# VanshJP/ShippingEnv

Measured on AMD Instinct MI355X. Metric: env-steps/sec at N=2^20 parallel envs per GPU (config 3: full step, 5 default ports; K steps in the steady state after a 1000-step pre-roll; config3_literal: the survey's 1000 steps from reset), higher is better.
Workload: dtype f64+int (fuel f64; reward computed in f64, stored f32 after one rounding; positions/cargo int)

## Files before the change

### shippingenv_amd/csrc/shipenv.hip

```cpp
#include <hip/hip_runtime.h>

#include <math.h>
#include <stdint.h>
#include <stdio.h>
#include <stdlib.h>
#include <string.h>

#include <algorithm>
#include <atomic>
#include <initializer_list>
#include <string>
#include <vector>

#include "../../include/shipenv.h"
#include "navfield.h"
#include "philox.h"
#include "step_lean.h"

#ifndef SHIPENV_TRACE
#define SHIPENV_TRACE 0
#endif

using namespace shipenv;

// ... 157 lines not shown
        double r = 0.0;
        if (k & 4) r += -10.0;
        if (k & 2) {
            r += -5.0;
        } else {
            r += -0.0001;
            r += -1.0;
        }
        r += (k & 1) ? 2.0 : -2.0;
        rtab[k] = r;
    }
    rtab[8] = 0.05;
    rtab[9] = 0.0;
    memcpy(&img[d.rtab()], rtab, sizeof rtab);
    dims = d;
    if (distinct) *distinct = ports_on_distinct_cells(P, px, py);
    return SE_OK;
}

int upload_world(se_env* env, int32_t P, const int32_t* px, const int32_t* py, const int32_t* pf,
                 const int32_t* pc) {
    WorldDims d{};
    std::vector<uint32_t> img;
    bool distinct = false;
    int rc = build_world_image(env->dims.H, env->dims.W, env->water, P, px, py, pf, pc, d, img, &distinct);
    if (rc) return rc;
    std::vector<uint8_t> ring(ring_table_bytes(d.H, d.W));
    ring_table_build(d.H, d.W, reinterpret_cast<const uint8_t*>(img.data()), ring.data());
    rc = device_reserve(env->d_world, env->world_cap, (size_t)d.padded() * 4 + ring.size());
    if (rc) return rc;
    HIP_TRY(hipMemcpy(env->d_world, img.data(), (size_t)d.padded() * 4, hipMemcpyHostToDevice));
    HIP_TRY(hipMemcpy(env->d_world + d.padded(), ring.data(), ring.size(), hipMemcpyHostToDevice));
    env->dims = d;
    env->ports_distinct = distinct;
    env->port_x.assign(px, px + P);
    env->port_y.assign(py, py + P);
    env->cmax = env->fmax = env->stock_cargo_max = 0;
    for (int i = 0; i < P; ++i) {
        env->cmax = std::max(env->cmax, std::min(pc[i], 49));
        env->fmax = std::max(env->fmax, std::min(pf[i], 199));
        env->stock_cargo_max = std::max(env->stock_cargo_max, pc[i]);
    }
    env->world_version += 1;
    env->mask_ntmpl = 1 + P;
    for (int p = 0; p < P; ++p)
        for (int q = 0; q < P; ++q) env->mask_ntmpl += (px[p] == px[q] && py[p] == py[q]) ? 1 : 0;
    return SE_OK;
}

typedef void (*StepFn)(StepArgs);
struct StepRow {
    uint32_t key;
    StepFn fn;
};
constexpr uint32_t step_key(bool typed, bool replay, bool autoreset, bool nt = false, bool rec = false, bool seq = false) {
    return typed | replay << 1 | autoreset << 2 | nt << 3 | rec << 4 | seq << 5;
}
template <bool... kFlags>
constexpr StepRow step_row() {
    return {step_key(kFlags...), step_kernel<kFlags...>};
}
template <bool... kFlags>
constexpr StepRow tail_row() {
    return {step_key(kFlags...), step_tail_kernel<kFlags...>};
}
constexpr StepRow kStepKernels[] = {
    step_row<false, false, false>(), step_row<false, false, false, true>(),
    step_row<false, false, true>(), step_row<false, false, true, true>(),
    step_row<false, false, false, false, false, true>(),
    step_row<false, false, false, true, false, true>(),
    step_row<false, false, true, false, true>(), step_row<false, false, true, true, true>(),
    step_row<false, true, false>(), step_row<true, true, false>(),
    step_row<true, false, false>(), step_row<true, false, true>(),
};
constexpr StepRow kStepTailKernels[] = {
    tail_row<false, false, false>(), tail_row<false, false, true>(), tail_row<false, true, false>(),
    tail_row<true, true, false>(),   tail_row<true, false, false>(), tail_row<true, false, true>(),
};

template <size_t kRows>
StepFn find_kernel(const StepRow (&rows)[kRows], uint32_t key) {
    for (const StepRow& r : rows)
        if (r.key == key) return r.fn;
    return nullptr;
}

StepArgs step_args(const se_env* env, const int32_t* act) {
    StepArgs A{};
    A.world = env->d_world;
    A.dims = env->dims;
    A.n = env->n;
    A.env_base = env->env_base;
    A.seed = env->seed;
    A.t = (uint32_t)env->step_t;
    A.st = env->st;
    A.act = act;
    A.iters = env->iters;
    return A;
}

int launch_step(se_env* env, bool typed, bool replay, const int32_t* act, const int32_t* a,
                const int32_t* b, se_tape* tape, void* stream, const StepRecord* rec = nullptr,
                bool seq = false) {
    int rc = check_ready(env);
    if (rc) return rc;
    if (env->n > 0 && (!act || (typed && (!a || !b)) || (replay && !tape)))
        return fail(SE_EINVAL, "null action/tape pointer");
    if (!aligned16(act) || (typed && (!aligned16(a) || !aligned16(b))))
        return fail(SE_EINVAL, "action buffers must be 16-byte aligned");
    const bool autoreset = (env->flags & SE_FLAG_AUTO_RESET) && !replay;
    if (autoreset && env->dims.P < 2) return fail(SE_EINVAL, "auto-reset needs at least two ports");
    DeviceGuard g(env->device);
    StepArgs A = step_args(env, act);
    A.act_a = a;
    A.act_b = b;
    A.tape = tape;
    if (autoreset) {
        const size_t par = (size_t)(env->step_t & 1u);
        A.done_recs = env->st.done_recs + par * (size_t)env->nseg * (size_t)env->seg;
        A.done_count = env->st.done_count + par * (size_t)env->nseg;
    }
    A.seg = env->seg;
    A.done_pad = env->done_pad;
    A.slab = env->d_slab;
    if (rec) A.rec = *rec;
    const bool agent = !typed && !replay;
    const StepFn full = find_kernel(kStepKernels, step_key(typed, replay, autoreset, agent && env->nt_loads,
                                                           rec != nullptr, agent && !autoreset && seq));
    const StepFn tail = find_kernel(kStepTailKernels, step_key(typed, replay, autoreset));
    if (!full || !tail) return fail(SE_EINVAL, "no step kernel for this kind of step");
    const hipStream_t s = (hipStream_t)stream;
    if (env->n >= kEnvsPerThread) {
        full<<<env->grid, kStepBlock, lds_bytes(env), s>>>(A);
        HIP_TRY(hipGetLastError());
    }
    if (env->n & 3) {
        tail<<<1, 64, 0, s>>>(A);
        HIP_TRY(hipGetLastError());
    }
    if (!replay) env->step_t += 1;
    return SE_OK;
}

int launch_step_seq(se_env* env, const int32_t* act, int64_t ld, int32_t steps, void* stream) {
    if (!act) return fail(SE_EINVAL, "null action/tape pointer");
    if (!aligned16(act)) return fail(SE_EINVAL, "action buffers must be 16-byte aligned");
    DeviceGuard g(env->device);
    const StepArgs A = step_args(env, act);
    const hipStream_t s = (hipStream_t)stream;
    if (env->n >= kEnvsPerThread) {
        const size_t base = lds_bytes(env) + kStockByCodeBytes;
        const bool pool = env->seq_gate_pool && base + kGatePoolBytes <= kLdsDefault;
        const size_t without = base + (pool ? kGatePoolBytes : 0);
        const uint32_t ring = env->seq_ring && ring_table_fits(env->dims.H, env->dims.W, env->dims.P, without)
                                  ? ring_table_bytes(env->dims.H, env->dims.W) : 0u;
        const size_t lds = without + ring;
        const auto kernel = pool ? (env->nt_loads ? step_seq_kernel<true, true> : step_seq_kernel<false, true>)
                                 : (env->nt_loads ? step_seq_kernel<true, false> : step_seq_kernel<false, false>);
        kernel<<<env->grid, kStepBlock, lds, s>>>(A, steps, ld, ring | (arrive_by_code_allowed(env->dims.P, env->ports_distinct) ? kSeqDistinctPorts : 0u), env->seq_screen ? 0u : ~0u);
        HIP_TRY(hipGetLastError());
    }
    if (env->n & 3) {
        step_tail_seq_kernel<<<1, 64, 0, s>>>(A, steps, ld);
        HIP_TRY(hipGetLastError());
    }
    env->step_t += (uint64_t)steps;
    return SE_OK;
}

int launch_reset(se_env* env, const uint8_t* mask, const int32_t* origin, const int32_t* dest, void* stream) {
    if (env->n == 0) return SE_OK;
    DeviceGuard g(env->device);
    const ResetArgs A{env->d_world, env->dims, env->n, env->env_base, env->seed,
                      (uint32_t)env->epoch, (uint32_t)env->step_t, env->st, mask, origin, dest};
    reset_kernel<<<grid_for(env->n), kBlock, 0, (hipStream_t)stream>>>(A);
    HIP_TRY(hipGetLastError());
    return SE_OK;
}

}

void shipenv_set_error(const std::string& msg) { g_err = msg; }

extern "C" {

#if SHIPENV_TRACE
extern "C" int se_trace_read(void* host, size_t bytes) {
    return hipMemcpyFromSymbol(host, HIP_SYMBOL(g_trace), bytes) == hipSuccess ? 0 : -1;
}
#endif

int se_abi_version(void) { return SHIPENV_ABI_VERSION; }

const char* se_last_error(void) { return g_err.c_str(); }

int se_create(se_env** out, int device, int64_t n, int64_t env_id_base, int32_t H, int32_t W,
              const uint8_t* water, int32_t P, const int32_t* port_x, const int32_t* port_y,
              const int32_t* port_fuel, const int32_t* port_cargo, uint64_t seed, uint32_t flags) {
    if (!out) return fail(SE_EINVAL, "null out");
    *out = nullptr;
    if (n < 0) return fail(SE_EINVAL, "n must be >= 0");
    if (env_id_base < 0 || (env_id_base & 3))
        return fail(SE_EINVAL, "env_id_base must be a multiple of 4 (envs 4k..4k+3 share draw blocks)");
    if (H < 1 || W < 1 || H > SE_MAX_SIDE || W > SE_MAX_SIDE)
        return fail(SE_EINVAL, "map sides must be in [1, 256]");
    if (!water) return fail(SE_EINVAL, "null water map");
    if (P > 0 && (!port_x || !port_y || !port_fuel || !port_cargo))
        return fail(SE_EINVAL, "null port arrays");
    int ndev = 0;
    HIP_TRY(hipGetDeviceCount(&ndev));
    if (device < 0 || device >= ndev) return fail(SE_EINVAL, "bad device ordinal");
    DeviceGuard g(device);
    se_env* env = new se_env();
    env->device = device;
    env->n = n;
    env->env_base = env_id_base;
    env->seed = seed;
    env->flags = flags;
    env->dims.H = H;
    env->dims.W = W;
    env->water.assign(water, water + (size_t)H * W);
    for (auto& v : env->water) v = v ? 1 : 0;
    int rc = upload_world(env, P, port_x, port_y, port_fuel, port_cargo);
    if (rc) {
        se_destroy(env);
        return rc;
    }
    {
        const int64_t groups = (n + kEnvsPerThread - 1) / kEnvsPerThread;
        const int64_t cap = step_block_cap();
        env->iters = groups > 0 ? (groups + cap * kStepBlock - 1) / (cap * kStepBlock) : 1;
        env->grid = (int)(groups > 0 ? (groups + env->iters * kStepBlock - 1) / (env->iters * kStepBlock) : 1);
        env->seg = 64 * kEnvsPerThread;
        env->nseg = (int64_t)env->grid * env->iters * (kStepBlock / 64);
        env->nslab = (int64_t)env->grid * (kStepBlock / 64);
        env->done_pad = done_pad_records(env);
        env->nt_loads = step_nt_loads(env);
        env->seq_fuse = seq_fuse();
        env->seq_max_steps = seq_max_steps();
        env->seq_gate_pool = seq_gate_pool();
        env->seq_ring = seq_ring();
        env->seq_screen = seq_screen();
        env->mask_tiled = mask_tiled();
    }
    hipError_t e = hipMalloc(&env->d_slab, (size_t)env->nslab * 4 * sizeof(double));
    if (e == hipSuccess) e = hipMemset(env->d_slab, 0, (size_t)env->nslab * 4 * sizeof(double));
    if (e != hipSuccess) {
        se_destroy(env);
        return fail(SE_EHIP, std::string("se_create allocation: ") + hipGetErrorString(e));
    }
    *out = env;
    return SE_OK;
}

int se_set_ports(se_env* env, int32_t P, const int32_t* port_x, const int32_t* port_y,
                 const int32_t* port_fuel, const int32_t* port_cargo) {
    if (!env) return fail(SE_EINVAL, "null env");
    if (P > 0 && (!port_x || !port_y || !port_fuel || !port_cargo))
        return fail(SE_EINVAL, "null port arrays");
    DeviceGuard g(env->device);
    HIP_TRY(hipDeviceSynchronize());
    return upload_world(env, P, port_x, port_y, port_fuel, port_cargo);
}

int se_bind(se_env* env, const se_state* st) {
    if (!env || !st) return fail(SE_EINVAL, "null argument");
    const void* req[] = {st->x, st->y, st->fuel, st->cargo, st->origin, st->dest,
                         st->reward, st->done, st->err};
    for (const void* p : req) {
        if (!p && env->n > 0) return fail(SE_EINVAL, "null state buffer");
        if (!aligned16(p)) return fail(SE_EINVAL, "state buffers must be 16-byte aligned");
    }
    if (env->flags & SE_FLAG_AUTO_RESET) {
        if ((env->n > 0 && (!st->ep_return || !st->ep_start)) || !st->done_recs || !st->done_count)
            return fail(SE_EINVAL, "auto-reset needs ep_return, ep_start, done_recs and done_count");
        if (!aligned16(st->ep_return) || !aligned16(st->ep_start) || !aligned16(st->done_recs))
            return fail(SE_EINVAL, "state buffers must be 16-byte aligned");
        DeviceGuard g(env->device);
        HIP_TRY(hipMemset(st->done_count, 0, 2 * (size_t)env->nseg * sizeof(int32_t)));
    }
    env->st = *st;
    env->bound = true;
    return SE_OK;
}

int se_reset(se_env* env, const uint8_t* mask, void* stream) {
    int rc = check_ready(env);
    if (rc) return rc;
    if (env->dims.P < 2) return fail(SE_EINVAL, "reset needs at least two ports");
    rc = launch_reset(env, mask, nullptr, nullptr, stream);
    if (rc) return rc;
    env->epoch += 1;
    return SE_OK;
}

int se_reset_to(se_env* env, const uint8_t* mask, const int32_t* origin, const int32_t* dest,
                void* stream) {
    int rc = check_ready(env);
    if (rc) return rc;
    if (env->n > 0 && (!origin || !dest)) return fail(SE_EINVAL, "null origin/dest");
    return launch_reset(env, mask, origin, dest, stream);
}

int se_step(se_env* env, const int32_t* actions, void* stream) {
    return launch_step(env, false, false, actions, nullptr, nullptr, nullptr, stream);
}

int se_step_seq_mark(se_env* env, const int32_t* actions, int64_t ld, int32_t steps, void* stream,
                     void* event, int32_t mark_after) {
    int rc = check_ready(env);
    if (rc) return rc;
    if (steps < 0) return fail(SE_EINVAL, "negative step count");
// ... 341 lines not shown
```

### shippingenv_amd/csrc/step_lean.h

```cpp
#pragma once
#include <hip/hip_runtime.h>
#include <math.h>
#include <stdint.h>

namespace shipenv {

__host__ __device__ __forceinline__ bool lean_do_move(int act, int P, bool nodest, bool inb) {
    const bool is_mv = (uint32_t)act + 4u < (P != 0 ? 8u : 0u);
    return is_mv & !nodest & inb;
}
__host__ __device__ __forceinline__ uint32_t lean_move_bound(int P) {
    return P != 0 ? 0xFFFFFFF7u : 0xFFFFFFFFu;
}
__host__ __device__ __forceinline__ bool lean_do_move_val(int val, uint32_t bound, bool nodest, bool inb) {
    const bool is_mv = (uint32_t)val > bound;
    return is_mv & !nodest & inb;
}
__host__ __device__ __forceinline__ bool lean_sel_ok(int act, int P, bool same) {
    const bool is_sel = (uint32_t)act - 4u < (uint32_t)P;
    return is_sel & !same;
}

constexpr uint32_t kRingBorder = 254;
constexpr uint32_t kRingGround = 255;
constexpr int kRingMaxPorts = 253;
constexpr size_t kRingLdsPerBlock = 160 * 1024 / 4;
constexpr uint32_t kRingBias = 0x00010001u;

__host__ __device__ __forceinline__ uint32_t ring_table_bytes(int H, int W) {
    return ((uint32_t)(H + 2) * (uint32_t)(W + 2) + 15u) & ~15u;
}
__host__ __device__ __forceinline__ bool ring_table_fits(int H, int W, int P, size_t lds_without) {
    return P <= kRingMaxPorts && lds_without + ring_table_bytes(H, W) <= kRingLdsPerBlock;
}
__host__ __forceinline__ void ring_table_build(int H, int W, const uint8_t* cell, uint8_t* out) {
    const uint32_t n = ring_table_bytes(H, W);
    for (uint32_t i = 0; i < n; ++i) out[i] = i < (uint32_t)(H + 2) * (uint32_t)(W + 2) ? (uint8_t)kRingBorder : 0;
    for (int x = 0; x < H; ++x)
        for (int y = 0; y < W; ++y) out[(size_t)(x + 1) * (size_t)(W + 2) + (size_t)(y + 1)] = cell[(size_t)x * W + y];
}
__host__ __device__ __forceinline__ uint32_t ring_bias(uint32_t p) { return p + kRingBias; }
__host__ __device__ __forceinline__ uint32_t ring_unbias(uint32_t bp) { return bp - kRingBias; }
__host__ __device__ __forceinline__ uint32_t ring_index(uint32_t bp, int W) {
    return (bp & 0xffffu) * (uint32_t)(W + 2) + (bp >> 16);
}
__host__ __device__ __forceinline__ bool ring_do_move(int val, uint32_t bound, uint32_t code) {
    return ((uint32_t)val > bound) & (code != kRingBorder);
}
__host__ __device__ __forceinline__ bool ring_moved(int val, uint32_t bound, uint32_t code) {
    return ((uint32_t)val > bound) & (code < kRingBorder);
}

__host__ __device__ __forceinline__ double lean_fuel(double fuel, double scale, bool moved) {
    return __builtin_fma(-scale, moved ? 1.0 : 0.0, fuel);
}

__host__ __device__ __forceinline__ double lean_fuel_scale(uint32_t w, double fifth) {
    return 1.0 + __builtin_fma((double)w, fifth, -0.1);
}

__host__ __device__ __forceinline__ uint32_t gate_window_log2(uint32_t m) {
    return m <= 8 ? 3u : m <= 16 ? 2u : 1u;
}

constexpr uint32_t kGatePoolLimit = 16;
constexpr uint32_t kGatePoolSeeds = 32;
constexpr uint32_t kGatePoolRow = 64 + kGatePoolSeeds;
constexpr uint32_t kGateWindowMax = 16;
constexpr uint32_t gate_window_entry_of(uint32_t m) {
    return m == 0 ? kGateWindowMax : (64u / m < kGateWindowMax ? 64u / m : kGateWindowMax) | ((65535u / m + 1u) << 8);
}
__host__ __device__ __forceinline__ uint32_t gate_window_entry(uint32_t m) {
    constexpr auto e = gate_window_entry_of;
    static constexpr uint32_t tab[17] = {e(0), e(1), e(2), e(3), e(4), e(5), e(6), e(7), e(8), e(9), e(10), e(11), e(12), e(13), e(14), e(15), e(16)};
    return tab[m];
}
__host__ __device__ __forceinline__ uint32_t gate_window_len(uint32_t entry) { return entry & 0xffu; }
__host__ __device__ __forceinline__ uint32_t gate_lane_offset(uint32_t L, uint32_t entry) { return (L * (entry >> 8)) >> 16; }
__host__ __device__ __forceinline__ uint32_t gate_lane_carrier(uint32_t L, uint32_t offset, uint32_t m) { return L - offset * m; }
__host__ __device__ __forceinline__ uint32_t gate_pool_index(uint32_t s, uint32_t m, uint32_t slot) { return s * m + slot; }
constexpr bool gate_pool_reads_in_rows() {
    for (uint32_t m = 1; m <= kGatePoolLimit; ++m) {
        const uint32_t W = gate_window_entry_of(m) & 0xffu;
        if (W < 4 || W > kGateWindowMax || m * W > 64 || (W - 1u) * m + m >= kGatePoolRow) return false;
    }
    return true;
}
__host__ __device__ __forceinline__ uint64_t gate_screen_mask(uint32_t m) { return m != 0 ? (1ull << m) - 1ull : ~0ull; }
__host__ __device__ __forceinline__ bool gate_screen_step(uint64_t shifted, uint64_t mask) { return (shifted & mask) != 0; }

__host__ __forceinline__ bool ports_on_distinct_cells(int P, const int32_t* px, const int32_t* py) {
    for (int i = 0; i < P; ++i)
        for (int k = 0; k < i; ++k)
            if (px[i] == px[k] && py[i] == py[k]) return false;
    return true;
}
__host__ __forceinline__ bool arrive_by_code_allowed(int P, bool distinct) { return distinct && P >= 2; }
__host__ __device__ __forceinline__ bool arrive_by_code(bool do_move, uint32_t code, int dst) {
    return do_move & (code == (uint32_t)dst + 1u);
}

__host__ __forceinline__ uint32_t gate_thr_entry(int c, double max_cargo) {
    return c < (int)max_cargo ? (uint32_t)floor(ldexp((double)c / max_cargo, 32)) : 0xffffffffu;
}

__host__ __device__ __forceinline__ bool screen_hot(const uint32_t word[4], const uint32_t thr[4]) {
    return (word[0] <= thr[0]) | (word[1] <= thr[1]) | (word[2] <= thr[2]) | (word[3] <= thr[3]);
}
__host__ __device__ __forceinline__ uint32_t screen_fold(uint64_t ballot, uint32_t logw) {
    uint32_t b = (uint32_t)ballot | (uint32_t)(ballot >> 32);
    b |= b >> 16;
    b |= b >> 8;
    b |= logw < 3u ? b >> 4 : 0u;
    b |= logw < 2u ? b >> 2 : 0u;
    return b;
}

}
```

### shippingenv_amd/csrc/step_seq.h

```cpp
#pragma once

#ifndef SHIPENV_SEQ_WINDOW_DIV
#define SHIPENV_SEQ_WINDOW_DIV 1
#endif
#ifndef SHIPENV_SEQ_CARGO_CUT
#define SHIPENV_SEQ_CARGO_CUT 1
#endif
#ifndef SHIPENV_SEQ_ARRIVE_CODE
#define SHIPENV_SEQ_ARRIVE_CODE 1
#endif

struct Carried {
    uint32_t pos[4];
    int org[4], dst[4];
    uint32_t code[4];
    bool near;
    bool bycode;
    uint32_t thr[4];
    const int2* take;
};
__device__ __forceinline__ uint32_t gate_thr_of(const LdsWorld& w, int cargo) {
    return w.gate_thr[min(max(cargo, 0), 50)];
}
template <bool kSched>
struct SeqInv {
    KeySched ks;
    uint32_t move_bound;
    uint32_t ring0;
    __device__ __forceinline__ U4 block(const Key& qk, uint32_t t, uint32_t slot) const {
        if constexpr (kSched) return draw_sched(ks, qk, t, slot);
        else return draw(qk, t, slot);
    }
};
struct NoLateDraw {
    __device__ __forceinline__ void operator()(U4&) const {}
};
template <bool kNt, bool kSched, typename Late = NoLateDraw>
__device__ __forceinline__ bool step_group_state(const LdsWorld& w, const SeqInv<kSched>& I, const Key& qk, uint32_t t, U4 fb,
                                                 const U4& gb, Group<false, false, kNt>& G, Carried& U, Late late = Late{}) {
    const int P = w.P;
    const uint32_t lim = (uint32_t)(w.H - 1) | ((uint32_t)(w.W - 1) << 16);
    const uint32_t wh = (uint32_t)w.W | (1u << 16);
    const uint32_t pm1 = P > 0 ? (uint32_t)(P - 1) : 0u;
    bool take_any = false;
#pragma unroll
    for (int j = 0; j < 4; ++j) take_any |= (G.a[j] >= 4 + P) & (U.code[j] != 0);
    const bool take_ran = __builtin_amdgcn_ballot_w64(take_any) != 0;
    if (take_ran) {
#pragma unroll
        for (int j = 0; j < 4; ++j) {
            const int act = G.a[j];
            const bool lt_tc = act < 54 + P;
            const int amount = act - (lt_tc ? 4 + P : 54 + P);
            const int2 st2 = U.take[U.code[j]];
            const int stock = lt_tc ? st2.y : st2.x;
            const bool ok_take = (act >= 4 + P) & (amount > 0) & (amount <= stock);
            G.c[j] = (ok_take & lt_tc) ? G.c[j] + amount : G.c[j];
            G.f[j] = (ok_take & !lt_tc) ? G.f[j] + (double)amount : G.f[j];
            U.thr[j] = gate_thr_of(w, G.c[j]);
        }
    }
    late(fb);
    uint32_t pos[4], cp[4], code_cp[4];
    int dst[4], cg[4];
    bool do_move[4], moved[4], inb[4], nodest[4];
#pragma unroll
    for (int j = 0; j < 4; ++j) {
        const uint32_t dxy = w.moves[G.a[j] & 3];
        const uint32_t p = U.pos[j];
        dst[j] = U.dst[j];
        const uint32_t np = pk_add_u16(p, dxy);
        inb[j] = pk_min_u16(np, lim) == np;
        nodest[j] = dst[j] == SE_NONE;
        cp[j] = (!nodest[j] & inb[j]) ? np : p;
        code_cp[j] = lds_cell(lds_address(w.cell), cp[j], wh);
    }
    asm("" : "+v"(code_cp[0]), "+v"(code_cp[1]), "+v"(code_cp[2]), "+v"(code_cp[3]));
#pragma unroll
    for (int j = 0; j < 4; ++j) {
        const int act = G.a[j];
        const int val = (int)((uint32_t)act - 4u);
        const uint32_t p = U.pos[j];
        cg[j] = G.c[j];
        const bool ground = code_cp[j] == kCellGround;
        const bool same = U.org[j] == val;
        do_move[j] = lean_do_move_val(val, I.move_bound, nodest[j], inb[j]);
        moved[j] = do_move[j] & !ground;
        const bool sel_ok = lean_sel_ok(act, P, same);
        pos[j] = moved[j] ? cp[j] : p;
        U.code[j] = moved[j] ? code_cp[j] : U.code[j];
        dst[j] = sel_ok ? val : dst[j];
    }
    uint32_t fire = 0, arrive = 0;
    bool arrive_any = false;
#pragma unroll
    for (int j = 0; j < 4; ++j) arrive_any |= do_move[j] & (U.code[j] != 0);
    if (__builtin_amdgcn_ballot_w64(arrive_any) != 0) {
#pragma unroll
        for (int j = 0; j < 4; ++j)
            arrive |= (uint32_t)(do_move[j] & (pos[j] == w.pos[min((uint32_t)dst[j], pm1)])) << j;
    }
    double f[4];
#pragma unroll
    for (int j = 0; j < 4; ++j) {
        f[j] = lean_fuel(G.f[j], lean_fuel_scale(fb.v[j], kFifthPerWord), moved[j]);
        const bool fires = do_move[j] & (cg[j] > 0) & (gb.v[j] <= U.thr[j]);
        fire |= (uint32_t)fires << j;
    }
    asm volatile("" : "+v"(fire), "+v"(arrive));
    int org[4];
#pragma unroll
    for (int j = 0; j < 4; ++j) {
        org[j] = U.org[j];
        U.pos[j] = pos[j];
        G.f[j] = f[j];
    }
    if (fire) {
        uint32_t lt[4], v1[4], v2[4], v3[4];
        const uint32_t rk[4] = {0u, fire & 1u, (uint32_t)__popc(fire & 3u), (uint32_t)__popc(fire & 7u)};
        U4 rr = I.block(qk, t, loss_slot(0));
#pragma unroll
        for (int j = 0; j < 4; ++j) {
            lt[j] = rr.v[0];
            v1[j] = rr.v[1];
            v2[j] = rr.v[2];
            v3[j] = rr.v[3];
        }
#pragma unroll
        for (uint32_t q = 1; q < 4; ++q) {
            if (__popc(fire) > q) {
                rr = I.block(qk, t, loss_slot(q));
#pragma unroll
                for (int j = (int)q; j < 4; ++j) {
                    const bool take = rk[j] >= q;
                    lt[j] = take ? rr.v[0] : lt[j];
                    v1[j] = take ? rr.v[1] : v1[j];
                    v2[j] = take ? rr.v[2] : v2[j];
                    v3[j] = take ? rr.v[3] : v3[j];
                }
            }
        }
#pragma unroll
        for (int j = 0; j < 4; ++j) {
            if (__builtin_amdgcn_ballot_w64((fire >> j) & 1u) == 0) continue;
            const uint32_t lo = min(v1[j], v2[j]), hi = max(v1[j], v2[j]);
            const uint32_t med = max(lo, min(hi, v3[j]));
            const int part = beta_part(med, cg[j]);
            const int some = lt[j] > kTypeHi ? cg[j] : part;
            const int loss = lt[j] < kTypeLo ? 0 : some;
            const bool fj = (fire >> j) & 1u;
            cg[j] = fj ? cg[j] - loss : cg[j];
            U.thr[j] = gate_thr_of(w, cg[j]);
        }
    }
    if (arrive) {
        const U4 ab = I.block(qk, t, kSlotArrive);
#pragma unroll
        for (int j = 0; j < 4; ++j) {
            const bool aj = (arrive >> j) & 1u;
            const int nd = pick_other(ab.v[j], P, dst[j]);
            cg[j] = aj ? 0 : cg[j];
            U.thr[j] = gate_thr_of(w, cg[j]);
            org[j] = aj ? dst[j] : org[j];
            dst[j] = aj ? nd : dst[j];
        }
    }
#pragma unroll
    for (int j = 0; j < 4; ++j) {
        U.org[j] = org[j];
        U.dst[j] = dst[j];
        G.c[j] = cg[j];
    }
    return take_ran;
}

struct GateDrawn {
    static constexpr bool kScreened = false;
    const U4& gb;
    __device__ __forceinline__ bool hot() const { return true; }
    __device__ __forceinline__ U4 words() const { return gb; }
};
__device__ __forceinline__ uint32_t here(uint32_t v) {
    asm volatile("" : "+v"(v));
    return v;
}
template <typename Read>
struct GateScreened {
    static constexpr bool kScreened = true;
    bool is_hot;
    Read read;
    __device__ __forceinline__ bool hot() const { return is_hot; }
    __device__ __forceinline__ U4 words() const { return read(); }
};
template <bool kNt, bool kSched, typename Gate, typename Late = NoLateDraw>
__device__ __forceinline__ bool step_group_ring(const LdsWorld& w, const SeqInv<kSched>& I, const Key& qk, uint32_t t, U4 fb,
                                                const Gate& gate, Group<false, false, kNt>& G, Carried& U, Late late = Late{}) {
    const int P = w.P;
    const uint32_t wh = (uint32_t)(w.W + 2) | (1u << 16);
    const uint32_t pm1 = P > 0 ? (uint32_t)(P - 1) : 0u;
    bool take_ran = false;
    if (U.near) {
        bool take_any = false;
#pragma unroll
        for (int j = 0; j < 4; ++j) take_any |= (G.a[j] >= 4 + P) & (U.code[j] != 0);
        take_ran = __builtin_amdgcn_ballot_w64(take_any) != 0;
        if (take_ran) {
            bool rose = false;
#pragma unroll
            for (int j = 0; j < 4; ++j) {
                const int act = G.a[j];
                const bool lt_tc = act < 54 + P;
                const int amount = act - (lt_tc ? 4 + P : 54 + P);
                const int2 st2 = U.take[U.code[j]];
                const int stock = lt_tc ? st2.y : st2.x;
                const bool ok_take = (act >= 4 + P) & (amount > 0) & (amount <= stock);
                rose |= ok_take & lt_tc;
                G.c[j] = (ok_take & lt_tc) ? G.c[j] + amount : G.c[j];
                G.f[j] = (ok_take & !lt_tc) ? G.f[j] + (double)amount : G.f[j];
                U.thr[j] = gate_thr_of(w, G.c[j]);
            }
#if SHIPENV_SEQ_CARGO_CUT
            take_ran = __builtin_amdgcn_ballot_w64(rose) != 0;
#else
            (void)rose;
#endif
        }
    }
    late(fb);
    uint32_t np[4], code_t[4];
#pragma unroll
    for (int j = 0; j < 4; ++j) {
        np[j] = pk_add_u16(U.pos[j], w.moves[G.a[j] & 3]);
        code_t[j] = lds_cell(I.ring0, np[j], wh);
    }
    asm("" : "+v"(code_t[0]), "+v"(code_t[1]), "+v"(code_t[2]), "+v"(code_t[3]));
    int dst[4], cg[4];
    bool do_move[4], moved[4], fires[4];
    double f[4];
#pragma unroll
    for (int j = 0; j < 4; ++j) {
        const int act = G.a[j];
        const int val = (int)((uint32_t)act - 4u);
        cg[j] = G.c[j];
        const bool same = U.org[j] == val;
        if constexpr (!Gate::kScreened) do_move[j] = ring_do_move(val, I.move_bound, code_t[j]);
        moved[j] = ring_moved(val, I.move_bound, code_t[j]);
        const bool sel_ok = lean_sel_ok(act, P, same);
        U.pos[j] = moved[j] ? np[j] : U.pos[j];
        U.code[j] = moved[j] ? code_t[j] : U.code[j];
        dst[j] = sel_ok ? val : U.dst[j];
        f[j] = lean_fuel(G.f[j], lean_fuel_scale(fb.v[j], kFifthPerWord), moved[j]);
        if constexpr (!Gate::kScreened) fires[j] = do_move[j] & (cg[j] > 0) & (gate.words().v[j] <= U.thr[j]);
    }
    const bool near = __builtin_amdgcn_ballot_w64((U.code[0] | U.code[1] | U.code[2] | U.code[3]) != 0) != 0;
    U.near = near;
    uint32_t arrive = 0;
    if (near) {
#pragma unroll
        for (int j = 0; j < 4; ++j)
            if constexpr (Gate::kScreened) do_move[j] = ring_do_move((int)((uint32_t)G.a[j] - 4u), I.move_bound, here(code_t[j]));
#if SHIPENV_SEQ_ARRIVE_CODE
        if (U.bycode) {
#pragma unroll
            for (int j = 0; j < 4; ++j) arrive |= (uint32_t)arrive_by_code(do_move[j], U.code[j], dst[j]) << j;
        } else
#endif
        {
#pragma unroll
            for (int j = 0; j < 4; ++j) arrive |= (uint32_t)(do_move[j] & (U.pos[j] == ring_bias(w.pos[min((uint32_t)dst[j], pm1)]))) << j;
        }
    }
    int org[4];
#pragma unroll
    for (int j = 0; j < 4; ++j) {
        org[j] = U.org[j];
        G.f[j] = f[j];
    }
    bool any_fire = false;
    if constexpr (Gate::kScreened) {
        if (gate.hot()) {
            const U4 gb = gate.words();
#pragma unroll
            for (int j = 0; j < 4; ++j)
                fires[j] = ring_do_move((int)((uint32_t)G.a[j] - 4u), I.move_bound, here(code_t[j])) & (cg[j] > 0) & (gb.v[j] <= U.thr[j]);
            any_fire = __builtin_amdgcn_ballot_w64(fires[0] | fires[1] | fires[2] | fires[3]) != 0;
        }
    } else {
        any_fire = __builtin_amdgcn_ballot_w64(fires[0] | fires[1] | fires[2] | fires[3]) != 0;
    }
    if (any_fire) {
        uint32_t fire = 0;
#pragma unroll
        for (int j = 0; j < 4; ++j) fire |= (uint32_t)fires[j] << j;
        asm volatile("" : "+v"(fire));
        uint32_t lt[4], v1[4], v2[4], v3[4];
        const uint32_t rk[4] = {0u, fire & 1u, (uint32_t)__popc(fire & 3u), (uint32_t)__popc(fire & 7u)};
        U4 rr = I.block(qk, t, loss_slot(0));
#pragma unroll
        for (int j = 0; j < 4; ++j) {
            lt[j] = rr.v[0];
            v1[j] = rr.v[1];
            v2[j] = rr.v[2];
            v3[j] = rr.v[3];
        }
#pragma unroll
        for (uint32_t q = 1; q < 4; ++q) {
            if (__popc(fire) > q) {
                rr = I.block(qk, t, loss_slot(q));
#pragma unroll
                for (int j = (int)q; j < 4; ++j) {
                    const bool take = rk[j] >= q;
                    lt[j] = take ? rr.v[0] : lt[j];
                    v1[j] = take ? rr.v[1] : v1[j];
                    v2[j] = take ? rr.v[2] : v2[j];
                    v3[j] = take ? rr.v[3] : v3[j];
                }
            }
        }
#pragma unroll
        for (int j = 0; j < 4; ++j) {
            if (__builtin_amdgcn_ballot_w64((fire >> j) & 1u) == 0) continue;
            const uint32_t lo = min(v1[j], v2[j]), hi = max(v1[j], v2[j]);
            const uint32_t med = max(lo, min(hi, v3[j]));
            const int part = beta_part(med, cg[j]);
            const int some = lt[j] > kTypeHi ? cg[j] : part;
            const int loss = lt[j] < kTypeLo ? 0 : some;
            const bool fj = (fire >> j) & 1u;
            cg[j] = fj ? cg[j] - loss : cg[j];
            U.thr[j] = gate_thr_of(w, cg[j]);
        }
    }
    if (arrive) {
        const U4 ab = I.block(qk, t, kSlotArrive);
#pragma unroll
        for (int j = 0; j < 4; ++j) {
            const bool aj = (arrive >> j) & 1u;
            const int nd = pick_other(ab.v[j], P, dst[j]);
            cg[j] = aj ? 0 : cg[j];
            U.thr[j] = gate_thr_of(w, cg[j]);
            org[j] = aj ? dst[j] : org[j];
            dst[j] = aj ? nd : dst[j];
        }
    }
#pragma unroll
    for (int j = 0; j < 4; ++j) {
        U.org[j] = org[j];
        U.dst[j] = dst[j];
        G.c[j] = cg[j];
    }
    return take_ran;
}

constexpr size_t kStockByCodeBytes = 256 * sizeof(int2);
static_assert(kStepBlock == 256, "stock_by_code: one cell code per thread");
__device__ __forceinline__ void stock_by_code(const LdsWorld& w, int2* take) {
    const uint32_t k = threadIdx.x - 1u, P = (uint32_t)w.P;
    const int2 s = w.stock[min(k, P > 0 ? P - 1 : 0u)];
    take[threadIdx.x] = k < P ? s : make_int2(0, 0);
}

constexpr uint32_t kGateDirectRun = 16;
constexpr uint32_t kGateEarlyCut = 2;
constexpr uint32_t kSeqDistinctPorts = 1;
static_assert(gate_pool_reads_in_rows(), "GATE pool: a window's reads lie in the wave's rows");
constexpr size_t kGatePoolBytes = (kStepBlock / 64) * kGatePoolRow * sizeof(uint4);
constexpr int kRingRows = 3;
static_assert(kGatePoolLimit <= kGatePoolSeeds && kGatePoolLimit <= 32, "GATE pool: a window of at least 2 steps");
static_assert(2 * kGatePoolLimit <= kGatePoolSeeds, "GATE pool: the carriers' threshold rows follow their seed rows");

template <bool kOpaque>
__device__ __forceinline__ uint32_t seq_lane() {
    uint32_t lane = threadIdx.x;
    if constexpr (kOpaque) asm volatile("" : "+v"(lane));
    return lane;
}

template <bool kNt, bool kPool>
__global__ __launch_bounds__(kStepBlock) __attribute__((amdgpu_waves_per_eu(4))) void step_seq_kernel(
    StepArgs A, int32_t steps, int64_t ld, uint32_t ring_bytes, uint32_t screen_all) {
    extern __shared__ uint32_t lds[];
    if (steps <= 0) return;
    const uint32_t ring16 = steps > 1 ? ring_bytes >> 4 : 0u;
    const bool has_ring = ring16 != 0;
    [[maybe_unused]] const bool distinct = (ring_bytes & kSeqDistinctPorts) != 0;
    const int64_t full = A.n >> 2;
    const int64_t first = (int64_t)blockIdx.x * A.iters * kStepBlock;

    const Staged st = stage_issue(A.world);
    __builtin_amdgcn_sched_barrier(0);
    Group<false, false, kNt> G;
    {
        const int64_t last = full - 1 - first;
        const uint32_t lane = last < (int64_t)threadIdx.x ? (uint32_t)(last < 0 ? 0 : last) : threadIdx.x;
        G.template load<true>(A, At<true>{last < 0 ? full - 1 : first, 0, A.n}, lane);
    }
    const uint4* const ring_g = reinterpret_cast<const uint4*>(A.world + A.dims.padded());
    const uint32_t ring_last = max(ring16, 1u) - 1u;
    const uint4 ring_r0 = ring_g[min(threadIdx.x, ring_last)];
    const uint4 ring_r1 = ring_g[min(threadIdx.x + kStepBlock, ring_last)];
    const uint4 ring_r2 = ring_g[min(threadIdx.x + 2 * kStepBlock, ring_last)];
    __builtin_amdgcn_sched_barrier(0);
    const LdsWorld w = stage_finish(A.world, A.dims, lds, st);
    int2* const take = reinterpret_cast<int2*>(lds + A.dims.padded());
    uint4* const gate_pool = reinterpret_cast<uint4*>(take + 256);
    uint4* const ring_l = reinterpret_cast<uint4*>(reinterpret_cast<uint8_t*>(take + 256) + (kPool ? kGatePoolBytes : 0));
    if (steps > 1) {
        stock_by_code(w, take);
        if (has_ring) {
            if (threadIdx.x < ring16) ring_l[threadIdx.x] = ring_r0;
            if (threadIdx.x + kStepBlock < ring16) ring_l[threadIdx.x + kStepBlock] = ring_r1;
            if (threadIdx.x + 2 * kStepBlock < ring16) ring_l[threadIdx.x + 2 * kStepBlock] = ring_r2;
            for (uint32_t i = threadIdx.x + kStepBlock * kRingRows; i < ring16; i += kStepBlock) ring_l[i] = ring_g[i];
        }
        __syncthreads();
    }

    SeqInv<kPool> I;
    if (steps > 1) {
        I.move_bound = lean_move_bound(w.P);
        asm volatile("" : "+s"(I.move_bound));
        I.ring0 = lds_address(reinterpret_cast<const uint8_t*>(ring_l));
    }

    BlockStats bs;
    Finished F;
    for (int64_t i = 0; i < A.iters; ++i) {
        const int64_t g0 = first + i * kStepBlock, g = g0 + threadIdx.x;
        if (g >= full) break;
        if (i > 0) {
            uint32_t lane = threadIdx.x;
            asm volatile("" : "+v"(lane));
            G.template load<true>(A, At<true>{g0, 0, A.n}, lane);
        }
        const uint32_t tl = A.t + (uint32_t)(steps - 1);
        if (steps > 1) {
            Carried U;
#pragma unroll
            for (int j = 0; j < 4; ++j) {
                U.pos[j] = unpack_pos(G.x, G.y, j);
                U.org[j] = byte_of(G.org, j);
                U.dst[j] = byte_of(G.dst, j);
                U.code[j] = w.cell[cell_of(U.pos[j], (uint32_t)w.W | (1u << 16))];
                U.thr[j] = gate_thr_of(w, G.c[j]);
            }
            U.take = take;
            bool irregular = false;
            {
                const uint32_t lim = (uint32_t)(w.H - 1) | ((uint32_t)(w.W - 1) << 16);
#pragma unroll
                for (int j = 0; j < 4; ++j) irregular |= (U.dst[j] == SE_NONE) | (pk_min_u16(U.pos[j], lim) != U.pos[j]);
            }
            const bool ring = has_ring && __builtin_amdgcn_ballot_w64(irregular) == 0;
            U.near = __builtin_amdgcn_ballot_w64((U.code[0] | U.code[1] | U.code[2] | U.code[3]) != 0) != 0;
            U.bycode = false;
#if SHIPENV_SEQ_ARRIVE_CODE
            if (distinct) {
                bool past = false;
#pragma unroll
                for (int j = 0; j < 4; ++j) past |= (uint32_t)U.dst[j] >= (uint32_t)w.P;
                U.bycode = __builtin_amdgcn_ballot_w64(past) == 0;
            }
#endif
            if (ring) {
#pragma unroll
                for (int j = 0; j < 4; ++j) U.pos[j] = ring_bias(U.pos[j]);
            }
            const Key qk = env_key(A.seed, (A.env_base + g * 4) >> 2);
            PairInv inv = pair_invariants(qk);
            asm volatile("" : "+v"(inv.hi[0]), "+v"(inv.lo[0]), "+v"(inv.hi[1]), "+v"(inv.lo[1]));
            const int32_t* row = A.act;
            if (!ring) {
                SeqInv<false> Ig;
                Ig.move_bound = I.move_bound;
                const uint32_t lane = seq_lane<kPool>();
                for (uint32_t t = A.t; t != tl; ++t) {
                    row += ld;
                    int32_t nxt[4];
                    ld4_full<kNt>(row, g0, nxt, lane);
                    const U4x2 fg = draw2(qk, inv, t);
                    step_group_state(w, Ig, qk, t, fg.fuel, fg.gate, G, U);
#pragma unroll
                    for (int j = 0; j < 4; ++j) G.a[j] = nxt[j];
                }
            } else if constexpr (!kPool) {
                for (uint32_t t = A.t; t != tl; ++t) {
                    row += ld;
                    int32_t nxt[4];
                    ld4_full<kNt>(row, g0, nxt);
                    const U4x2 fg = draw2(qk, inv, t);
                    step_group_ring(w, I, qk, t, fg.fuel, GateDrawn{fg.gate}, G, U);
#pragma unroll
                    for (int j = 0; j < 4; ++j) G.a[j] = nxt[j];
                }
            } else {
                {
                    const Key sk = env_key(A.seed, 0);
                    I.ks = key_schedule(sk.k0, sk.k1);
                    pin_schedule(I.ks);
                }
                const uint32_t lane = seq_lane<true>(), L = lane & 63u;
                uint4* const pool = gate_pool + (lane >> 6) * kGatePoolRow;
                uint4* const seeds = pool + 64;
                const bool whole = __builtin_amdgcn_ballot_w64(true) == ~0ull;
                uint32_t cuts = 0;
                for (uint32_t t = A.t; t != tl;) {
                    bool pooled = true;
                    do {
                        const bool carry = (G.c[0] > 0) | (G.c[1] > 0) | (G.c[2] > 0) | (G.c[3] > 0);
                        const uint64_t M = __builtin_amdgcn_ballot_w64(carry);
                        const uint32_t m = (uint32_t)__popcll(M);
                        if (!whole || m > kGatePoolLimit || (cuts >= 2 && m != 0)) {
                            pooled = false;
                            break;
                        }
                        const uint32_t slot = __builtin_amdgcn_mbcnt_hi((uint32_t)(M >> 32), __builtin_amdgcn_mbcnt_lo((uint32_t)M, 0u));
#if SHIPENV_SEQ_WINDOW_DIV
                        const uint32_t went = gate_window_entry(m);
                        uint64_t screen = (uint64_t)(int64_t)(int32_t)screen_all;
                        const uint64_t smask = gate_screen_mask(m);
                        if (m != 0) {
                            if (carry) {
                                seeds[slot] = make_uint4(inv.c3, inv.hi[1], inv.lo[1], qk.e1);
                                seeds[kGatePoolLimit + slot] = make_uint4(U.thr[0], U.thr[1], U.thr[2], U.thr[3]);
                            }
                            __builtin_amdgcn_fence(__ATOMIC_RELEASE, "wavefront");
                            __builtin_amdgcn_wave_barrier();
                            __builtin_amdgcn_fence(__ATOMIC_ACQUIRE, "wavefront");
                            const uint32_t so = gate_lane_offset(L, went), of = gate_lane_carrier(L, so, m);
                            const uint4 sd = seeds[of];
                            const uint4 th = seeds[kGatePoolLimit + of];
                            const U4 gw = draw_gate_pooled_sched(I.ks, GateSeed{sd.x, sd.y, sd.z, sd.w}, t + so);
                            pool[L] = make_uint4(gw.v[0], gw.v[1], gw.v[2], gw.v[3]);
                            screen |= __builtin_amdgcn_ballot_w64(gw.v[0] <= th.x) | __builtin_amdgcn_ballot_w64(gw.v[1] <= th.y) |
                                      __builtin_amdgcn_ballot_w64(gw.v[2] <= th.z) | __builtin_amdgcn_ballot_w64(gw.v[3] <= th.w);
                            __builtin_amdgcn_fence(__ATOMIC_RELEASE, "wavefront");
                            __builtin_amdgcn_wave_barrier();
                            __builtin_amdgcn_fence(__ATOMIC_ACQUIRE, "wavefront");
                        }
                        const uint32_t win = m != 0 ? min(tl - t, gate_window_len(went)) : tl - t;
                        uint32_t s = 0;
                        bool took;
                        do {
                            row += ld;
                            int32_t nxt[4];
                            ld4_full<kNt>(row, g0, nxt, lane);
                            const auto words = [&]() {
                                uint32_t so = s;
                                asm volatile("" : "+s"(so));
                                const uint4 g4 = pool[gate_pool_index(so, m, slot)];
                                return U4{{g4.x, g4.y, g4.z, g4.w}};
                            };
                            const auto fuel = [&](U4& fb) {
                                fb = draw_fuel_sched(I.ks, qk, inv, t);
                                asm volatile("" : "+v"(fb.v[0]), "+v"(fb.v[1]), "+v"(fb.v[2]), "+v"(fb.v[3]));
                            };
                            took = step_group_ring(w, I, qk, t, U4{}, GateScreened<decltype(words)>{gate_screen_step(screen, smask), words}, G, U, fuel);
#pragma unroll
                            for (int j = 0; j < 4; ++j) G.a[j] = nxt[j];
                            screen >>= m;
                            ++s;
                            ++t;
                        } while (!took && s != win);
#else
                        const uint32_t logw = gate_window_log2(m);
                        const uint32_t wmask = (1u << logw) - 1u;
                        uint32_t screen = screen_all;
                        if (m != 0) {
                            if (carry) {
                                seeds[slot] = make_uint4(inv.c3, inv.hi[1], inv.lo[1], qk.e1);
                                seeds[kGatePoolLimit + slot] = make_uint4(U.thr[0], U.thr[1], U.thr[2], U.thr[3]);
                            }
                            __builtin_amdgcn_fence(__ATOMIC_RELEASE, "wavefront");
                            __builtin_amdgcn_wave_barrier();
                            __builtin_amdgcn_fence(__ATOMIC_ACQUIRE, "wavefront");
                            const uint32_t of = min(L >> logw, m - 1u);
                            const uint4 sd = seeds[of];
                            const uint4 th = seeds[kGatePoolLimit + of];
                            const U4 gw = draw_gate_pooled_sched(I.ks, GateSeed{sd.x, sd.y, sd.z, sd.w}, t + (L & wmask));
                            pool[L] = make_uint4(gw.v[0], gw.v[1], gw.v[2], gw.v[3]);
                            const uint64_t hot = __builtin_amdgcn_ballot_w64(gw.v[0] <= th.x) | __builtin_amdgcn_ballot_w64(gw.v[1] <= th.y) |
                                                 __builtin_amdgcn_ballot_w64(gw.v[2] <= th.z) | __builtin_amdgcn_ballot_w64(gw.v[3] <= th.w);
                            screen |= screen_fold(hot, logw);
                            __builtin_amdgcn_fence(__ATOMIC_RELEASE, "wavefront");
                            __builtin_amdgcn_wave_barrier();
                            __builtin_amdgcn_fence(__ATOMIC_ACQUIRE, "wavefront");
                        }
                        const uint4* const mine = pool + ((slot << logw) & 63u);
                        const uint32_t win = m != 0 ? min(tl - t, wmask + 1u) : tl - t;
                        uint32_t s = 0;
                        bool took;
                        do {
                            row += ld;
                            int32_t nxt[4];
                            ld4_full<kNt>(row, g0, nxt, lane);
                            const auto words = [&]() {
                                const uint4 g4 = mine[s & wmask];
                                return U4{{g4.x, g4.y, g4.z, g4.w}};
                            };
                            const auto fuel = [&](U4& fb) {
                                fb = draw_fuel_sched(I.ks, qk, inv, t);
                                asm volatile("" : "+v"(fb.v[0]), "+v"(fb.v[1]), "+v"(fb.v[2]), "+v"(fb.v[3]));
                            };
                            took = step_group_ring(w, I, qk, t, U4{}, GateScreened<decltype(words)>{((screen >> (s & 31u)) & 1u) != 0, words}, G, U, fuel);
#pragma unroll
                            for (int j = 0; j < 4; ++j) G.a[j] = nxt[j];
                            ++s;
                            ++t;
                        } while (!took && s != win);
#endif
                        cuts = took && m != 0 && s <= kGateEarlyCut ? cuts + 1u : 0u;
                    } while (t != tl);
                    if (pooled) break;
                    cuts = min(cuts, 1u);
                    for (uint32_t n = min(tl - t, kGateDirectRun); n != 0; --n, ++t) {
                        row += ld;
                        int32_t nxt[4];
                        ld4_full<kNt>(row, g0, nxt, lane);
                        const U4x2 fg = draw2(qk, inv, t);
                        step_group_ring(w, I, qk, t, fg.fuel, GateDrawn{fg.gate}, G, U);
#pragma unroll
                        for (int j = 0; j < 4; ++j) G.a[j] = nxt[j];
                    }
                }
            }
            if (ring) {
#pragma unroll
                for (int j = 0; j < 4; ++j) U.pos[j] = ring_unbias(U.pos[j]);
            }
            pack_pos(U.pos, G.x, G.y);
            G.org = G.dst = 0;
#pragma unroll
            for (int j = 0; j < 4; ++j) {
                G.org |= (uint32_t)(U.org[j] & 0xff) << (8 * j);
                G.dst |= (uint32_t)(U.dst[j] & 0xff) << (8 * j);
            }
        }
        StepOut O;
        const uint32_t ln = seq_lane<true>();
        const At<true> at{g0, (g0 + ln) * 4, A.n};
        step_group_agent<false, true, kNt, false, false, true>(A, w, G, at, bs, F, early_draws<false>(A, at.base, tl), tl, &O);
        const se_state& S = late_args().st;
        __builtin_amdgcn_sched_barrier(0);
        st4u8_full(S.x, g0, G.x, ln);
        st4u8_full(S.y, g0, G.y, ln);
        st4_full(S.fuel, g0, G.f, ln);
        st4u8_full(S.done, g0, O.dn, ln);
        st4u8_full(reinterpret_cast<uint8_t*>(S.err), g0, O.ee, ln);
        __builtin_amdgcn_sched_barrier(0);
        st4u8_full(S.origin, g0, G.org, ln);
        st4u8_full(S.dest, g0, G.dst, ln);
        st4_full(S.cargo, g0, G.c, ln);
        st4_full(S.reward, g0, O.rw, ln);
    }
}

__global__ __launch_bounds__(64) void step_tail_seq_kernel(StepArgs A, int32_t steps, int64_t ld) {
    if (threadIdx.x != 0) return;
    const LdsWorld w = world_view(A.dims, A.world);
    const int32_t* act = A.act;
    const uint32_t t0 = A.t;
    for (int32_t k = 0; k < steps; ++k) {
        A.act = act + (int64_t)k * ld;
        A.t = t0 + (uint32_t)k;
        step_tail_envs<false, false, false>(A, w);
    }
}
```

Baseline: 827.3 billion.

## Carry ship positions as LDS byte addresses in ring-table step loop

Ship positions inside the sequential step loop are kept as direct LDS byte addresses into the padded ring table, not as packed (x,y) u16 pairs. Each move becomes one signed byte delta read from a small LDS table, and the cell lookup needs no index multiply. Port positions are converted into the same address space with udot2 for the arrival compare, and positions are converted back with a reciprocal-multiply unindex at the end. This cuts per-step ALU work for address computation at the cost of an extra LDS delta read per move and more kernel template variants.

```diff
diff --git a/shippingenv_amd/csrc/shipenv.hip b/shippingenv_amd/csrc/shipenv.hip
--- a/shippingenv_amd/csrc/shipenv.hip
+++ b/shippingenv_amd/csrc/shipenv.hip
@@ -333,12 +333,19 @@
         const size_t base = lds_bytes(env) + kStockByCodeBytes;
         const bool pool = env->seq_gate_pool && base + kGatePoolBytes <= kLdsDefault;
         const size_t without = base + (pool ? kGatePoolBytes : 0);
-        const uint32_t ring = env->seq_ring && ring_table_fits(env->dims.H, env->dims.W, env->dims.P, without)
+        const uint32_t ring = env->seq_ring && ring_table_fits(env->dims.H, env->dims.W, env->dims.P, without + kSeqDeltaBytes)
                                   ? ring_table_bytes(env->dims.H, env->dims.W) : 0u;
-        const size_t lds = without + ring;
-        const auto kernel = pool ? (env->nt_loads ? step_seq_kernel<true, true> : step_seq_kernel<false, true>)
-                                 : (env->nt_loads ? step_seq_kernel<true, false> : step_seq_kernel<false, false>);
-        kernel<<<env->grid, kStepBlock, lds, s>>>(A, steps, ld, ring | (arrive_by_code_allowed(env->dims.P, env->ports_distinct) ? kSeqDistinctPorts : 0u), env->seq_screen ? 0u : ~0u);
+        const size_t lds = without + ring + (ring ? kSeqDeltaBytes : 0);
+        const bool addr = SHIPENV_SEQ_CELL_ADDR && ring != 0 && ring_byte_deltas(env->dims.W);
+        auto kernel = pool ? (env->nt_loads ? step_seq_kernel<true, true, false> : step_seq_kernel<false, true, false>)
+                           : (env->nt_loads ? step_seq_kernel<true, false, false> : step_seq_kernel<false, false, false>);
+#if SHIPENV_SEQ_CELL_ADDR
+        if (addr)
+            kernel = pool ? (env->nt_loads ? step_seq_kernel<true, true, true> : step_seq_kernel<false, true, true>)
+                          : (env->nt_loads ? step_seq_kernel<true, false, true> : step_seq_kernel<false, false, true>);
+#endif
+        kernel<<<env->grid, kStepBlock, lds, s>>>(A, steps, ld, ring | (arrive_by_code_allowed(env->dims.P, env->ports_distinct) ? kSeqDistinctPorts : 0u), env->seq_screen ? 0u : ~0u,
+                                                  addr ? ring_unindex_mul(env->dims.W) : 0u);
         HIP_TRY(hipGetLastError());
     }
     if (env->n & 3) {
diff --git a/shippingenv_amd/csrc/step_lean.h b/shippingenv_amd/csrc/step_lean.h
--- a/shippingenv_amd/csrc/step_lean.h
+++ b/shippingenv_amd/csrc/step_lean.h
@@ -49,6 +49,17 @@
 }
 __host__ __device__ __forceinline__ bool ring_moved(int val, uint32_t bound, uint32_t code) {
     return ((uint32_t)val > bound) & (code < kRingBorder);
+}
+
+constexpr size_t kRingDeltaBytes = 16;
+__host__ __device__ __forceinline__ bool ring_byte_deltas(int W) { return W + 2 <= 127; }
+__host__ __device__ __forceinline__ int ring_delta(uint32_t mv, int W) {
+    return (int)(int16_t)(mv & 0xffffu) * (W + 2) + (int)(int16_t)(mv >> 16);
+}
+__host__ __device__ __forceinline__ uint32_t ring_unindex_mul(int W) { return 0xffffffffu / (uint32_t)(W + 2) + 1u; }
+__host__ __device__ __forceinline__ uint32_t ring_unindex(uint32_t index, int W, uint32_t mul) {
+    const uint32_t q = (uint32_t)(((uint64_t)index * mul) >> 32);
+    return q | ((index - q * (uint32_t)(W + 2)) << 16);
 }
 
 __host__ __device__ __forceinline__ double lean_fuel(double fuel, double scale, bool moved) {
diff --git a/shippingenv_amd/csrc/step_seq.h b/shippingenv_amd/csrc/step_seq.h
--- a/shippingenv_amd/csrc/step_seq.h
+++ b/shippingenv_amd/csrc/step_seq.h
@@ -8,6 +8,9 @@
 #endif
 #ifndef SHIPENV_SEQ_ARRIVE_CODE
 #define SHIPENV_SEQ_ARRIVE_CODE 1
+#endif
+#ifndef SHIPENV_SEQ_CELL_ADDR
+#define SHIPENV_SEQ_CELL_ADDR 1
 #endif
 
 struct Carried {
@@ -27,6 +30,7 @@
     KeySched ks;
     uint32_t move_bound;
     uint32_t ring0;
+    uint32_t delta0;
     __device__ __forceinline__ U4 block(const Key& qk, uint32_t t, uint32_t slot) const {
         if constexpr (kSched) return draw_sched(ks, qk, t, slot);
         else return draw(qk, t, slot);
@@ -192,7 +196,13 @@
     __device__ __forceinline__ bool hot() const { return is_hot; }
     __device__ __forceinline__ U4 words() const { return read(); }
 };
-template <bool kNt, bool kSched, typename Gate, typename Late = NoLateDraw>
+typedef __attribute__((address_space(3))) const int8_t lds_i8;
+typedef uint32_t u32x2 __attribute__((ext_vector_type(2)));
+typedef __attribute__((address_space(3))) const u32x2 lds_u32x2;
+__device__ __forceinline__ uint32_t ring_address(uint32_t ring0, uint32_t bp, uint32_t wh) {
+    return __builtin_amdgcn_udot2(__builtin_bit_cast(u16x2, bp), __builtin_bit_cast(u16x2, wh), ring0, false);
+}
+template <bool kAddr, bool kNt, bool kSched, typename Gate, typename Late = NoLateDraw>
 __device__ __forceinline__ bool step_group_ring(const LdsWorld& w, const SeqInv<kSched>& I, const Key& qk, uint32_t t, U4 fb,
                                                 const Gate& gate, Group<false, false, kNt>& G, Carried& U, Late late = Late{}) {
     const int P = w.P;
@@ -230,8 +240,14 @@
     uint32_t np[4], code_t[4];
 #pragma unroll
     for (int j = 0; j < 4; ++j) {
-        np[j] = pk_add_u16(U.pos[j], w.moves[G.a[j] & 3]);
-        code_t[j] = lds_cell(I.ring0, np[j], wh);
+        if constexpr (kAddr) {
+            const int8_t d = *(lds_i8*)(uintptr_t)(((uint32_t)G.a[j] & 3u) | I.delta0);
+            np[j] = U.pos[j] + (uint32_t)(int32_t)d;
+            code_t[j] = *(lds_u8*)(uintptr_t)np[j];
+        } else {
+            np[j] = pk_add_u16(U.pos[j], w.moves[G.a[j] & 3]);
+            code_t[j] = lds_cell(I.ring0, np[j], wh);
+        }
     }
     asm("" : "+v"(code_t[0]), "+v"(code_t[1]), "+v"(code_t[2]), "+v"(code_t[3]));
     int dst[4], cg[4];
@@ -266,8 +282,14 @@
         } else
 #endif
         {
-#pragma unroll
-            for (int j = 0; j < 4; ++j) arrive |= (uint32_t)(do_move[j] & (U.pos[j] == ring_bias(w.pos[min((uint32_t)dst[j], pm1)]))) << j;
+            [[maybe_unused]] u32x2 rw = {0u, 0u};
+            if constexpr (kAddr) rw = *(lds_u32x2*)(uintptr_t)(I.delta0 + 8u);
+#pragma unroll
+            for (int j = 0; j < 4; ++j) {
+                uint32_t port = ring_bias(w.pos[min((uint32_t)dst[j], pm1)]);
+                if constexpr (kAddr) port = ring_address(rw.x, port, rw.y);
+                arrive |= (uint32_t)(do_move[j] & (U.pos[j] == port)) << j;
+            }
         }
     }
     int org[4];
@@ -365,6 +387,7 @@
 static_assert(gate_pool_reads_in_rows(), "GATE pool: a window's reads lie in the wave's rows");
 constexpr size_t kGatePoolBytes = (kStepBlock / 64) * kGatePoolRow * sizeof(uint4);
 constexpr int kRingRows = 3;
+constexpr size_t kSeqDeltaBytes = SHIPENV_SEQ_CELL_ADDR ? kRingDeltaBytes : 0;
 static_assert(kGatePoolLimit <= kGatePoolSeeds && kGatePoolLimit <= 32, "GATE pool: a window of at least 2 steps");
 static_assert(2 * kGatePoolLimit <= kGatePoolSeeds, "GATE pool: the carriers' threshold rows follow their seed rows");
 
@@ -375,9 +398,9 @@
     return lane;
 }
 
-template <bool kNt, bool kPool>
+template <bool kNt, bool kPool, bool kAddr>
 __global__ __launch_bounds__(kStepBlock) __attribute__((amdgpu_waves_per_eu(4))) void step_seq_kernel(
-    StepArgs A, int32_t steps, int64_t ld, uint32_t ring_bytes, uint32_t screen_all) {
+    StepArgs A, int32_t steps, int64_t ld, uint32_t ring_bytes, uint32_t screen_all, uint32_t ring_inv) {
     extern __shared__ uint32_t lds[];
     if (steps <= 0) return;
     const uint32_t ring16 = steps > 1 ? ring_bytes >> 4 : 0u;
@@ -411,6 +434,11 @@
             if (threadIdx.x + kStepBlock < ring16) ring_l[threadIdx.x + kStepBlock] = ring_r1;
             if (threadIdx.x + 2 * kStepBlock < ring16) ring_l[threadIdx.x + 2 * kStepBlock] = ring_r2;
             for (uint32_t i = threadIdx.x + kStepBlock * kRingRows; i < ring16; i += kStepBlock) ring_l[i] = ring_g[i];
+            if constexpr (kAddr) {
+                if (threadIdx.x < 4) reinterpret_cast<int8_t*>(ring_l + ring16)[threadIdx.x] = (int8_t)ring_delta(w.moves[threadIdx.x], w.W);
+                if (threadIdx.x == 4)
+                    reinterpret_cast<uint2*>(ring_l + ring16)[1] = make_uint2(lds_address(reinterpret_cast<const uint8_t*>(ring_l)), (uint32_t)(w.W + 2) | (1u << 16));
+            }
         }
         __syncthreads();
     }
@@ -420,6 +448,7 @@
         I.move_bound = lean_move_bound(w.P);
         asm volatile("" : "+s"(I.move_bound));
         I.ring0 = lds_address(reinterpret_cast<const uint8_t*>(ring_l));
+        I.delta0 = lds_address(reinterpret_cast<const uint8_t*>(ring_l + ring16));
     }
 
     BlockStats bs;
@@ -463,7 +492,10 @@
 #endif
             if (ring) {
 #pragma unroll
-                for (int j = 0; j < 4; ++j) U.pos[j] = ring_bias(U.pos[j]);
+                for (int j = 0; j < 4; ++j) {
+                    U.pos[j] = ring_bias(U.pos[j]);
+                    if constexpr (kAddr) U.pos[j] = ring_address(I.ring0, U.pos[j], (uint32_t)(w.W + 2) | (1u << 16));
+                }
             }
             const Key qk = env_key(A.seed, (A.env_base + g * 4) >> 2);
             PairInv inv = pair_invariants(qk);
@@ -488,7 +520,7 @@
                     int32_t nxt[4];
                     ld4_full<kNt>(row, g0, nxt);
                     const U4x2 fg = draw2(qk, inv, t);
-                    step_group_ring(w, I, qk, t, fg.fuel, GateDrawn{fg.gate}, G, U);
+                    step_group_ring<kAddr>(w, I, qk, t, fg.fuel, GateDrawn{fg.gate}, G, U);
 #pragma unroll
                     for (int j = 0; j < 4; ++j) G.a[j] = nxt[j];
                 }
@@ -554,7 +586,7 @@
                                 fb = draw_fuel_sched(I.ks, qk, inv, t);
                                 asm volatile("" : "+v"(fb.v[0]), "+v"(fb.v[1]), "+v"(fb.v[2]), "+v"(fb.v[3]));
                             };
-                            took = step_group_ring(w, I, qk, t, U4{}, GateScreened<decltype(words)>{gate_screen_step(screen, smask), words}, G, U, fuel);
+                            took = step_group_ring<kAddr>(w, I, qk, t, U4{}, GateScreened<decltype(words)>{gate_screen_step(screen, smask), words}, G, U, fuel);
 #pragma unroll
                             for (int j = 0; j < 4; ++j) G.a[j] = nxt[j];
                             screen >>= m;
@@ -601,7 +633,7 @@
                                 fb = draw_fuel_sched(I.ks, qk, inv, t);
                                 asm volatile("" : "+v"(fb.v[0]), "+v"(fb.v[1]), "+v"(fb.v[2]), "+v"(fb.v[3]));
                             };
-                            took = step_group_ring(w, I, qk, t, U4{}, GateScreened<decltype(words)>{((screen >> (s & 31u)) & 1u) != 0, words}, G, U, fuel);
+                            took = step_group_ring<kAddr>(w, I, qk, t, U4{}, GateScreened<decltype(words)>{((screen >> (s & 31u)) & 1u) != 0, words}, G, U, fuel);
 #pragma unroll
                             for (int j = 0; j < 4; ++j) G.a[j] = nxt[j];
                             ++s;
@@ -617,7 +649,7 @@
                         int32_t nxt[4];
                         ld4_full<kNt>(row, g0, nxt, lane);
                         const U4x2 fg = draw2(qk, inv, t);
-                        step_group_ring(w, I, qk, t, fg.fuel, GateDrawn{fg.gate}, G, U);
+                        step_group_ring<kAddr>(w, I, qk, t, fg.fuel, GateDrawn{fg.gate}, G, U);
 #pragma unroll
                         for (int j = 0; j < 4; ++j) G.a[j] = nxt[j];
                     }
@@ -625,7 +657,10 @@
             }
             if (ring) {
 #pragma unroll
-                for (int j = 0; j < 4; ++j) U.pos[j] = ring_unbias(U.pos[j]);
+                for (int j = 0; j < 4; ++j) {
+                    if constexpr (kAddr) U.pos[j] = ring_unindex(U.pos[j] - I.ring0, w.W, ring_inv);
+                    U.pos[j] = ring_unbias(U.pos[j]);
+                }
             }
             pack_pos(U.pos, G.x, G.y);
             G.org = G.dst = 0;
```

After: 874.3 billion (median of 6 runs). 1.06x the previous value.
